# thomasahle/tinyknn

Measured on AMD Instinct MI355X. Metric: queries/sec at Recall10@10 on GloVe-100 angular (synthetic stand-in), IVF+4-bit PQ, build_probes=1, higher is better.
Workload: dtype int8 (saturating PQ sums) + f32 (tables, rescoring); 1 GPU; glove-100-angular stand-in: 300 Gaussian clusters sigma 0.7, N=1183514 d=100 IVF n_clusters=1087 build_probes=1 FastPQ dpb=2 M=52; k=10, n_probes=10, parallelism=replica x1 (queries sharded), batches_in_flight=2

## Files before the change

tinyknn_amd/csrc/plain_scan.hip:

```cpp
#include <limits.h>
#include <stdlib.h>

#include "kernels.h"
#include "tickets.h"

typedef int v4i __attribute__((ext_vector_type(4)));
typedef int v16i __attribute__((ext_vector_type(16)));

#ifdef TK_PLAIN_CLOCK
__device__ unsigned long long tk_plain_clock[4];
#define TK_CLOCK_BEGIN() const unsigned long long ck_t0_ = __builtin_readcyclecounter(), ck_r0_ = __builtin_amdgcn_s_memrealtime()
#define TK_CLOCK_END()                                                                          \
    do {                                                                                        \
        if ((threadIdx.x & 63) == 0) {                                                          \
            atomicAdd(&tk_plain_clock[0], (unsigned long long)__builtin_readcyclecounter() - ck_t0_);       \
            atomicAdd(&tk_plain_clock[1], (unsigned long long)__builtin_amdgcn_s_memrealtime() - ck_r0_);   \
            atomicAdd(&tk_plain_clock[2], 1ull);                                                \
        }                                                                                       \
    } while (0)
#else
#define TK_CLOCK_BEGIN()
#define TK_CLOCK_END()
#endif
#ifdef TK_PLAIN_STAMPS
__device__ unsigned long long tk_plain_stamps[8];
#define TK_STAMP(i)                                                   \
    do {                                                              \
        const unsigned long long now_ = __builtin_readcyclecounter(); \
        stamp_acc[i] += now_ - stamp_last;                            \
        stamp_last = now_;                                            \
    } while (0)
#else
#define TK_STAMP(i)
#endif

__global__ __launch_bounds__(256) void table_limits_kernel(const uint4 *__restrict__ tables, int M_used,
                                                           int M, int avx, int64_t nq, int force,
                                                           int *__restrict__ qlim)
{
    const int lane = threadIdx.x & 63;
    const int64_t q = (int64_t)blockIdx.x * 4 + (threadIdx.x >> 6);
    if (q >= nq) return;
    int n0 = 0, n1 = 0;
    for (int m = lane; m < M_used; m += 64) {
        const uint4 t = tables[q * M + m];
        const uint32_t w[4] = {t.x, t.y, t.z, t.w};
        int mn = 127;
#pragma unroll
        for (int i = 0; i < 4; i++)
#pragma unroll
            for (int b = 0; b < 4; b++) {
                const int v = (int)(int8_t)(w[i] >> (8 * b));
                mn = v < mn ? v : mn;
            }
        const int neg = mn < 0 ? -mn : 0;
        if (avx && ((m >> 1) & 1)) n1 += neg; else n0 += neg;
    }
    for (int o = 32; o > 0; o >>= 1) {
        n0 += __shfl_xor(n0, o, 64);
        n1 += __shfl_xor(n1, o, 64);
    }
    if (lane == 0) {
        int c = (n0 <= 128 && n1 <= 128) ? 127 - n0 - n1 : TK_PLAIN_NEVER;
        if (force != INT_MAX && c > force) c = force;
        qlim[q] = c;
    }
}


void tk_launch_table_limits(const uint4 *tables, int M, int order, int64_t nq, int *qlim, hipStream_t s, int force)
{
    if (nq == 0) return;
    const int avx = order == TK_ORDER_AVX;
    const int M_used = avx ? (M & ~3) : M;
    hipLaunchKernelGGL(table_limits_kernel, dim3((unsigned)((nq + 3) / 4)), dim3(256), 0, s, tables,
                       M_used, M, avx, nq, force, qlim);
}

__device__ __forceinline__ uint32_t pack4(int a, int b, int c, int d)
{
    const uint32_t lo = __builtin_amdgcn_perm((uint32_t)b, (uint32_t)a, 0x0c0c0400u);
    const uint32_t hi = __builtin_amdgcn_perm((uint32_t)d, (uint32_t)c, 0x04000c0cu);
    return lo | hi;
}

__device__ __forceinline__ int clamp8(int x) { return min(max(x, -128), 127); }

typedef __attribute__((address_space(3))) const v4i lds_cv4i;
__device__ __forceinline__ v4i one_hot(uint32_t lut0, uint32_t x, uint32_t rot)
{
    const uint32_t a = (__builtin_amdgcn_alignbit(x, x, rot) & 0xf0u) | lut0;
    return *(lds_cv4i *)(uintptr_t)a;
}

__device__ __forceinline__ void swap_halves(uint32_t &a, uint32_t &b)
{
    auto r = __builtin_amdgcn_permlane32_swap(a, b, false, false);
    a = r[0];
    b = r[1];
}

template <int PT>
struct PlainWaveShape {
    static constexpr int PS = (PT + 3) & ~3;
    static constexpr size_t wave_out = 32 * 9 * 16 + 32 * 8 + 2 * 32 * 8;
    static constexpr size_t lds = 256 + (size_t)4 * 8 * PS * 4 + 4 * wave_out;
};

template <int PT, bool EXACT>
__global__ __launch_bounds__(256, 2) void scan_plain_wave_kernel(TkScanJob j, int P, int M)
{
    if (EXACT) P = PT;
    TK_CLOCK_BEGIN();
#ifdef TK_PLAIN_STAMPS
    unsigned long long stamp_acc[6] = {0, 0, 0, 0, 0, 0}, stamp_last = __builtin_readcyclecounter(), stamp_it = 0;
    const unsigned long long stamp_k0 = stamp_last;
#endif
    using SH = PlainWaveShape<PT>;
    constexpr int PS = SH::PS;
    extern __shared__ __attribute__((aligned(256))) unsigned char smem_plain[];
    uint4 *lut = (uint4 *)smem_plain;
    uint32_t *stage = (uint32_t *)(smem_plain + 256);
    const int lane = threadIdx.x & 63, wave = threadIdx.x >> 6;
    unsigned char *wout = smem_plain + 256 + 4 * 8 * PS * 4 + wave * SH::wave_out;
    uint4 *otile = (uint4 *)wout;
    uint8_t *omin = wout + 32 * 9 * 16;
    long long *orow = (long long *)(wout + 32 * 9 * 16 + 32 * 8);
    long long *omrow = orow + 32;
    if (threadIdx.x < 16) {
        uint32_t w[4] = {0, 0, 0, 0};
        w[threadIdx.x >> 2] = 1u << (8 * (threadIdx.x & 3));
        lut[threadIdx.x] = make_uint4(w[0], w[1], w[2], w[3]);
    }
    __syncthreads();
    const int n_units = j.unit_prefix[j.n_lists];
    int *ticket = const_cast<int *>(j.unit_prefix) + TK_TICKET_OFF(j.n_lists);
    const int r = lane & 31, h = lane >> 5;
    const int rr = r & 15;
    const uint32_t rot = (uint32_t)(8 * (rr & 3) + 4 * h + 28) & 31u;
    const uint32_t lut0 = (uint32_t)(uintptr_t)(__attribute__((address_space(3))) unsigned char *)smem_plain;
    const bool loader = lane < 2 * P;
    const int ll = loader ? lane : 2 * P - 1;
    const int lch = ll / P, lp = ll - lch * P;
    uint32_t *st = stage + wave * 8 * PS;
    uint32_t *stw = st + (lch * 4) * PS + lp;
    const uint32_t *rd = st + ((r >> 4) * 4 + (rr >> 2)) * PS;

    ticketed_blocks(n_units, ticket, [&](int u) {
        TK_STAMP(5);
        const int4 d = ((const int4 *)j.unit_desc4)[u];
        const int l = __builtin_amdgcn_readfirstlane(d.x), t = __builtin_amdgcn_readfirstlane(d.y);
        const int cpa = __builtin_amdgcn_readfirstlane(d.z), cpb = __builtin_amdgcn_readfirstlane(d.w);
        const int po = j.pair_off[l];
        int nvalid = j.pair_off[l + 1] - po - 32 * t;
        nvalid = nvalid < 32 ? nvalid : 32;
        const int rec = po + 32 * t + (r < nvalid ? r : nvalid - 1);
        const int qi = j.pair_q[rec], f0 = j.pair_f0[rec];
        const int64_t c0 = j.list_chunk_off[l];
        const int C = (int)(j.list_chunk_off[l + 1] - c0);
        const uint4 *cbase = j.codes + (c0 >> 3) * (int64_t)(8 * P) + lp * 8;
        const int cin = (int)(c0 & 7);
        auto fetch = [&](int cp) -> uint4 {
            int c = 2 * cp + lch;
            c = (c < C ? c : C - 1) + cin;
            return cbase[(c >> 3) * (8 * P) + (c & 7)];
        };
        uint4 ga = fetch(cpa), gb = fetch(cpa + 1);
        v4i B[PT];
        {
            const v4i *brow = (const v4i *)(j.tables + (int64_t)qi * M + h);
#pragma unroll
            for (int p = 0; p < PT; p++) B[p] = (EXACT || p < P) ? brow[2 * p] : v4i{0, 0, 0, 0};
        }
        if (h == 0) {
            orow[r] = (long long)qi * j.cap + f0;
            omrow[r] = (long long)qi * j.min_stride + f0;
        }
        const int c_end = 2 * cpb < C ? 2 * cpb : C;

        auto stage_codes = [&](const uint4 g) {
            if (loader) {
                stw[0 * PS] = g.x;
                stw[1 * PS] = g.y;
                stw[2 * PS] = g.z;
                stw[3 * PS] = g.w;
            }
        };
        auto flush = [&](int g8) {
            __builtin_amdgcn_fence(__ATOMIC_RELEASE, "wavefront");
            __builtin_amdgcn_wave_barrier();
            const int s = lane & 7, chunk = 8 * g8 + s;
            const bool cok = chunk >= 2 * cpa && chunk < c_end;
#pragma unroll
            for (int k = 0; k < 4; k++) {
                const int qq = (lane >> 3) + 8 * k;
                const uint4 v = otile[qq * 9 + s];
                const uint8_t m = omin[qq * 8 + s];
                const long long ro = orow[qq], mo = omrow[qq];
                if (cok && qq < nvalid) {
                    j.dist[ro + chunk] = v;
                    j.mins[mo + chunk] = m;
                }
            }
            __builtin_amdgcn_fence(__ATOMIC_ACQUIRE, "wavefront");
            __builtin_amdgcn_wave_barrier();
        };
        TK_STAMP(0);
        auto chunk_pair = [&](int cp) {
            TK_STAMP(1);
            __builtin_amdgcn_fence(__ATOMIC_RELEASE, "wavefront");
            __builtin_amdgcn_wave_barrier();
            v16i acc = {0, 0, 0, 0, 0, 0, 0, 0, 0, 0, 0, 0, 0, 0, 0, 0};
            uint32_t x[PS];
#pragma unroll
            for (int k = 0; k < PS / 4; k++) {
                const uint4 v = *(const uint4 *)(rd + 4 * k);
                x[4 * k] = v.x; x[4 * k + 1] = v.y; x[4 * k + 2] = v.z; x[4 * k + 3] = v.w;
            }
            v4i A[PT];
#pragma unroll
            for (int p = 0; p < PT; p++) A[p] = one_hot(lut0, x[p], rot);
#pragma unroll
            for (int p = 0; p < PT; p++)
                acc = __builtin_amdgcn_mfma_i32_32x32x32_i8(A[p], B[p], acc, 0, 0, 0);
            constexpr int DEPTH = 6 < PT ? 6 : PT;
            __builtin_amdgcn_sched_group_barrier(0x100, PS / 4 + DEPTH, 0);
#pragma unroll
            for (int p = 0; p < PT - DEPTH; p++) {
                __builtin_amdgcn_sched_group_barrier(0x008, 1, 0);
                __builtin_amdgcn_sched_group_barrier(0x100, 1, 0);
            }
            __builtin_amdgcn_sched_group_barrier(0x008, DEPTH, 0);
            __builtin_amdgcn_fence(__ATOMIC_ACQUIRE, "wavefront");
            __builtin_amdgcn_wave_barrier();
            int o[16];
#pragma unroll
            for (int i = 0; i < 16; i++) o[i] = clamp8(acc[i]);
#ifdef TK_PLAIN_STAMPS
            asm volatile("s_nop 0" ::"v"(o[15]));
            TK_STAMP(2);
            stamp_it++;
#endif
            uint32_t X = pack4(o[0], o[1], o[2], o[3]), Y = pack4(o[4], o[5], o[6], o[7]);
            uint32_t Z = pack4(o[8], o[9], o[10], o[11]), W = pack4(o[12], o[13], o[14], o[15]);
            uint32_t mA = (uint32_t)min(min(min(o[0], o[1]), min(o[2], o[3])), min(min(o[4], o[5]), min(o[6], o[7])));
            uint32_t mB = (uint32_t)min(min(min(o[8], o[9]), min(o[10], o[11])), min(min(o[12], o[13]), min(o[14], o[15])));
            swap_halves(X, Z);
            swap_halves(Y, W);
            swap_halves(mA, mB);
            const int mn = min((int)mA, (int)mB);
            const int slot = (2 * cp + h) & 7;
            otile[r * 9 + slot] = make_uint4(X, Z, Y, W);
            omin[r * 8 + slot] = (uint8_t)mn;
            TK_STAMP(3);
            if ((cp & 3) == 3) flush(cp >> 2);
            TK_STAMP(4);
        };
#define TK_PAIR(cp_)                                  \
        {                                             \
            stage_codes(ga);                          \
            ga = fetch((cp_) + 2);                    \
            chunk_pair(cp_);                          \
            stage_codes(gb);                          \
            gb = fetch((cp_) + 3);                    \
            chunk_pair((cp_) + 1);                    \
        }
        int cp = cpa;
        if (cp + 1 < cpb) {
            TK_PAIR(cp)
            cp += 2;
#pragma nounroll
            while (cp + 1 < cpb) {
                TK_PAIR(cp)
                cp += 2;
            }
        }
#undef TK_PAIR
        if (cp < cpb) {
            stage_codes(ga);
            chunk_pair(cp);
            cp++;
        }
        if ((cp & 3) != 0) flush((cp - 1) >> 2);
        TK_STAMP(4);
    });
    TK_CLOCK_END();
#ifdef TK_PLAIN_STAMPS
    if (lane == 0) {
        for (int i = 0; i < 6; i++) atomicAdd(&tk_plain_stamps[i], stamp_acc[i]);
        atomicAdd(&tk_plain_stamps[6], stamp_it);
        atomicAdd(&tk_plain_stamps[7], (unsigned long long)__builtin_readcyclecounter() - stamp_k0);
    }
#endif
}

int tk_plain_fits(int M) { return M >= 2 && M % 2 == 0 && M / 2 <= 26; }

int tk_launch_scan_plain(const TkScanJob &j, int M, int order, int n_blocks, hipStream_t s)
{
    if (!j.unit_prefix) return 0;
    int P = M / 2;
    if (order == TK_ORDER_AVX) P &= ~1;
    if (P < 1 || P > 26) return -1;
#define TK_LAUNCH_W(PT_, EX_)                                                                       \
    do {                                                                                            \
        static bool attr_ = false;                                                                  \
        if (!attr_) {                                                                               \
            if (hipFuncSetAttribute((const void *)scan_plain_wave_kernel<PT_, EX_>,           \
                                    hipFuncAttributeMaxDynamicSharedMemorySize,                     \
                                    (int)PlainWaveShape<PT_>::lds) != hipSuccess)                   \
                return -1;                                                                          \
            attr_ = true;                                                                           \
        }                                                                                           \
        hipLaunchKernelGGL((scan_plain_wave_kernel<PT_, EX_>), dim3(n_blocks), dim3(256),     \
                           PlainWaveShape<PT_>::lds, s, j, P, M);                                   \
    } while (0)
    if (P == 26) TK_LAUNCH_W(26, true);
    else if (P == 16) TK_LAUNCH_W(16, true);
    else if (P <= 8) TK_LAUNCH_W(8, false);
    else if (P <= 16) TK_LAUNCH_W(16, false);
    else TK_LAUNCH_W(26, false);
#undef TK_LAUNCH_W
    return 0;
}
```

Measured before the change: 25.71 million queries/s.

## Transpose scan outputs in registers via DPP/permlane instead of LDS tile

The per-wave LDS output tile used to stage dist/min results before global stores is removed. Results from four chunk pairs are now held in registers and transposed with permlane32 swaps and DPP quad swaps, so each lane writes its rows directly. The MFMA loop is also rescheduled with explicit sched_barriers that interleave the one-hot LDS reads and the staged-code reads with the matrix ops. This cuts LDS traffic and footprint, which may allow more occupancy, at the cost of extra VGPRs for the buffered outputs and more permute instructions.

```diff
diff --git a/tinyknn_amd/csrc/plain_scan.hip b/tinyknn_amd/csrc/plain_scan.hip
--- a/tinyknn_amd/csrc/plain_scan.hip
+++ b/tinyknn_amd/csrc/plain_scan.hip
@@ -103,9 +103,20 @@
 template <int PT>
 struct PlainWaveShape {
     static constexpr int PS = (PT + 3) & ~3;
-    static constexpr size_t wave_out = 32 * 9 * 16 + 32 * 8 + 2 * 32 * 8;
+    static constexpr size_t wave_out = 2 * 32 * 8;
     static constexpr size_t lds = 256 + (size_t)4 * 8 * PS * 4 + 4 * wave_out;
+    static constexpr int DEPTH = 6 < PT ? 6 : PT;
+    static constexpr int X_FIRST = 4 < PS / 4 ? 4 : PS / 4;
 };
+static_assert(PlainWaveShape<26>::lds <= 6 * 1024, "the plain kernel keeps its outputs out of LDS");
+
+template <int CTRL>
+__device__ __forceinline__ void swap_quad(uint32_t &a, uint32_t &b, bool up)
+{
+    const uint32_t t = (uint32_t)__builtin_amdgcn_mov_dpp((int)(up ? a : b), CTRL, 0xf, 0xf, true);
+    a = up ? t : a;
+    b = up ? b : t;
+}
 
 template <int PT, bool EXACT>
 __global__ __launch_bounds__(256, 2) void scan_plain_wave_kernel(TkScanJob j, int P, int M)
@@ -122,10 +133,7 @@
     uint4 *lut = (uint4 *)smem_plain;
     uint32_t *stage = (uint32_t *)(smem_plain + 256);
     const int lane = threadIdx.x & 63, wave = threadIdx.x >> 6;
-    unsigned char *wout = smem_plain + 256 + 4 * 8 * PS * 4 + wave * SH::wave_out;
-    uint4 *otile = (uint4 *)wout;
-    uint8_t *omin = wout + 32 * 9 * 16;
-    long long *orow = (long long *)(wout + 32 * 9 * 16 + 32 * 8);
+    long long *orow = (long long *)(smem_plain + 256 + 4 * 8 * PS * 4 + wave * SH::wave_out);
     long long *omrow = orow + 32;
     if (threadIdx.x < 16) {
         uint32_t w[4] = {0, 0, 0, 0};
@@ -177,6 +185,7 @@
             omrow[r] = (long long)qi * j.min_stride + f0;
         }
         const int c_end = 2 * cpb < C ? 2 * cpb : C;
+        uint32_t cur[2][5] = {{0, 0, 0, 0, 0}, {0, 0, 0, 0, 0}}, lo[2][5] = {{0, 0, 0, 0, 0}, {0, 0, 0, 0, 0}};
 
         auto stage_codes = [&](const uint4 g) {
             if (loader) {
@@ -186,51 +195,62 @@
                 stw[3 * PS] = g.w;
             }
         };
-        auto flush = [&](int g8) {
-            __builtin_amdgcn_fence(__ATOMIC_RELEASE, "wavefront");
-            __builtin_amdgcn_wave_barrier();
-            const int s = lane & 7, chunk = 8 * g8 + s;
+        auto flush = [&](int g8, uint32_t (&b0)[5], uint32_t (&b1)[5], uint32_t (&b2)[5], uint32_t (&b3)[5]) {
+            int ln = lane;
+            asm volatile("" : "+v"(ln));
+#pragma unroll
+            for (int w = 0; w < 5; w++) {
+                swap_halves(b0[w], b2[w]);
+                swap_halves(b1[w], b3[w]);
+                swap_quad<0xb1>(b0[w], b2[w], ln & 1);
+                swap_quad<0xb1>(b1[w], b3[w], ln & 1);
+                swap_quad<0x4e>(b0[w], b1[w], ln & 2);
+                swap_quad<0x4e>(b2[w], b3[w], ln & 2);
+            }
+            const int chunk = 8 * g8 + 4 * (lane >> 5) + (lane & 3);
             const bool cok = chunk >= 2 * cpa && chunk < c_end;
-#pragma unroll
-            for (int k = 0; k < 4; k++) {
-                const int qq = (lane >> 3) + 8 * k;
-                const uint4 v = otile[qq * 9 + s];
-                const uint8_t m = omin[qq * 8 + s];
+            auto put = [&](int qq, const uint32_t (&v)[5]) {
                 const long long ro = orow[qq], mo = omrow[qq];
                 if (cok && qq < nvalid) {
-                    j.dist[ro + chunk] = v;
-                    j.mins[mo + chunk] = m;
+                    j.dist[ro + chunk] = make_uint4(v[0], v[1], v[2], v[3]);
+                    j.mins[mo + chunk] = (uint8_t)v[4];
                 }
-            }
-            __builtin_amdgcn_fence(__ATOMIC_ACQUIRE, "wavefront");
-            __builtin_amdgcn_wave_barrier();
+            };
+            put((r & 28) + 0, b0);
+            put((r & 28) + 2, b1);
+            put((r & 28) + 1, b2);
+            put((r & 28) + 3, b3);
+            TK_STAMP(4);
         };
         TK_STAMP(0);
-        auto chunk_pair = [&](int cp) {
+        auto chunk_pair = [&](int cp, uint32_t (&out)[5]) {
             TK_STAMP(1);
             __builtin_amdgcn_fence(__ATOMIC_RELEASE, "wavefront");
             __builtin_amdgcn_wave_barrier();
             v16i acc = {0, 0, 0, 0, 0, 0, 0, 0, 0, 0, 0, 0, 0, 0, 0, 0};
             uint32_t x[PS];
-#pragma unroll
-            for (int k = 0; k < PS / 4; k++) {
+            auto read_x = [&](int k) {
                 const uint4 v = *(const uint4 *)(rd + 4 * k);
                 x[4 * k] = v.x; x[4 * k + 1] = v.y; x[4 * k + 2] = v.z; x[4 * k + 3] = v.w;
-            }
+            };
+            constexpr int DEPTH = SH::DEPTH, XF = SH::X_FIRST;
+            constexpr int XP = 4 * XF - DEPTH - 4 > 0 ? 4 * XF - DEPTH - 4 : 0;
             v4i A[PT];
 #pragma unroll
-            for (int p = 0; p < PT; p++) A[p] = one_hot(lut0, x[p], rot);
-#pragma unroll
-            for (int p = 0; p < PT; p++)
+            for (int k = 0; k < XF; k++) read_x(k);
+#pragma unroll
+            for (int p = 0; p < DEPTH; p++) A[p] = one_hot(lut0, x[p], rot);
+#pragma unroll
+            for (int p = 0; p < PT; p++) {
+                __builtin_amdgcn_sched_barrier(0);
                 acc = __builtin_amdgcn_mfma_i32_32x32x32_i8(A[p], B[p], acc, 0, 0, 0);
-            constexpr int DEPTH = 6 < PT ? 6 : PT;
-            __builtin_amdgcn_sched_group_barrier(0x100, PS / 4 + DEPTH, 0);
-#pragma unroll
-            for (int p = 0; p < PT - DEPTH; p++) {
-                __builtin_amdgcn_sched_group_barrier(0x008, 1, 0);
-                __builtin_amdgcn_sched_group_barrier(0x100, 1, 0);
-            }
-            __builtin_amdgcn_sched_group_barrier(0x008, DEPTH, 0);
+                if (p == XP) {
+#pragma unroll
+                    for (int k = XF; k < PS / 4; k++) read_x(k);
+                }
+                if (p + DEPTH < PT) A[p + DEPTH] = one_hot(lut0, x[p + DEPTH], rot);
+            }
+            __builtin_amdgcn_sched_barrier(0);
             __builtin_amdgcn_fence(__ATOMIC_ACQUIRE, "wavefront");
             __builtin_amdgcn_wave_barrier();
             int o[16];
@@ -248,22 +268,24 @@
             swap_halves(X, Z);
             swap_halves(Y, W);
             swap_halves(mA, mB);
-            const int mn = min((int)mA, (int)mB);
-            const int slot = (2 * cp + h) & 7;
-            otile[r * 9 + slot] = make_uint4(X, Z, Y, W);
-            omin[r * 8 + slot] = (uint8_t)mn;
+            out[0] = X; out[1] = Z; out[2] = Y; out[3] = W;
+            out[4] = (uint32_t)min((int)mA, (int)mB);
             TK_STAMP(3);
-            if ((cp & 3) == 3) flush(cp >> 2);
-            TK_STAMP(4);
         };
-#define TK_PAIR(cp_)                                  \
-        {                                             \
-            stage_codes(ga);                          \
-            ga = fetch((cp_) + 2);                    \
-            chunk_pair(cp_);                          \
-            stage_codes(gb);                          \
-            gb = fetch((cp_) + 3);                    \
-            chunk_pair((cp_) + 1);                    \
+#define TK_PAIR(cp_)                                                             \
+        {                                                                        \
+            stage_codes(ga);                                                     \
+            ga = fetch((cp_) + 2);                                               \
+            chunk_pair(cp_, cur[0]);                                             \
+            stage_codes(gb);                                                     \
+            gb = fetch((cp_) + 3);                                               \
+            chunk_pair((cp_) + 1, cur[1]);                                       \
+            if ((cp_) & 2) flush((cp_) >> 2, lo[0], lo[1], cur[0], cur[1]);      \
+            else                                                                 \
+                for (int w = 0; w < 5; w++) {                                    \
+                    lo[0][w] = cur[0][w];                                        \
+                    lo[1][w] = cur[1][w];                                        \
+                }                                                                \
         }
         int cp = cpa;
         if (cp + 1 < cpb) {
@@ -278,11 +300,12 @@
 #undef TK_PAIR
         if (cp < cpb) {
             stage_codes(ga);
-            chunk_pair(cp);
-            cp++;
-        }
-        if ((cp & 3) != 0) flush((cp - 1) >> 2);
-        TK_STAMP(4);
+            chunk_pair(cp, cur[0]);
+            if (cp & 2) flush(cp >> 2, lo[0], lo[1], cur[0], cur[1]);
+            else flush(cp >> 2, cur[0], cur[1], lo[0], lo[1]);
+        } else if (cp & 2) {
+            flush(cp >> 2, lo[0], lo[1], cur[0], cur[1]);
+        }
     });
     TK_CLOCK_END();
 #ifdef TK_PLAIN_STAMPS
```

Result: slower. 23.40 million queries/s (-9.0%).
